# cure-lab/MagicDrive

Measured on AMD Instinct MI355X. Metric: 6-view scenes/sec at 224x400, 50-step DDIM, higher is better.
Workload: dtype bf16; 1 GPU; configs[1]: 6-view 224x400, text-only conditioning (camera_param=None -> CFG off), 50-step DDIM, bf16; scenes_per_gpu=64, ddim_steps=50, scheduler=ddim, parallelism=scene-sharded x1, hipgraph=True, streams=2, output_type=latent

## Files before the change

### include/mdx.h

```cpp
#ifndef MDX_H_
#define MDX_H_

#include <stdint.h>

#ifdef __cplusplus
extern "C" {
#endif

#define MDX_OK 0
#define MDX_EINVAL (-1)
#define MDX_ELAUNCH (-2)
#define MDX_EUNSUPPORTED (-3)

#define MDX_ABI_VERSION 12

#define MDX_EPI_NONE 0
#define MDX_EPI_GEGLU 1
#define MDX_EPI_SILU 2

typedef struct MdxGemmDesc {
    const void* A; const void* W; void* C; const void* R;
    const float* bias; const float* temb; const int32_t* sel_ptr; float* ws;
    int64_t M, N, K;
    int64_t lda, ldw, ldc, ldr;
// ... 46 lines not shown
    int64_t ldq, sQ, ldk, sK, ldv, sV, ldo, sO;
    double scale;
    int64_t joint;
    int64_t q_prescaled;
    int64_t causal;
    int64_t v_rowmajor;
} MdxAttnDesc;
int mdx_attention_bf16(const MdxAttnDesc* d, void* stream);

typedef struct MdxGroupNormDesc {
    const void* X; void* Y; const float* gamma; const float* beta;
    int64_t B, HW, C, G, ldx, ldy;
    double eps;
    int64_t silu;
    float* ws; int64_t ws_bytes;
} MdxGroupNormDesc;
int mdx_groupnorm_bf16(const MdxGroupNormDesc* d, void* stream);

typedef struct MdxLayerNormDesc {
    const void* X; void* Y; const float* gamma; const float* beta;
    int64_t M, C, ldx, ldy;
    double eps;
    int64_t reserved0;
} MdxLayerNormDesc;
int mdx_layernorm_bf16(const MdxLayerNormDesc* d, void* stream);

typedef struct MdxSoftmaxDesc {
    const float* X; void* Y;
    int64_t rows, T, ldx, ldy;
    double scale;
    int64_t reserved0;
} MdxSoftmaxDesc;
// ... 116 lines not shown
```

### magicdrive_amd/_lib.py

```python
from __future__ import annotations

import ctypes as C
import os
from typing import Dict, List, Tuple

_HERE = os.path.dirname(os.path.abspath(__file__))
LIB_PATH = os.environ.get("MDX_LIB_PATH") or os.path.join(_HERE, "libmdx.so")

ABI_VERSION = 12

OP_GEMM, OP_CONV, OP_CONV_DIRECT, OP_ATTN, OP_GROUPNORM, OP_LAYERNORM = 1, 2, 3, 4, 5, 6
OP_EW, OP_FOURIER, OP_GATHER, OP_TIMEEMB, OP_DDIM, OP_UNIPC, OP_SOFTMAX = 7, 8, 9, 10, 11, 12, 13
OP_BYTES = 512

EPI_NONE, EPI_GEGLU, EPI_SILU = 0, 1, 2
EW_ADD, EW_COPY, EW_UPSAMPLE, EW_NCHW_TO_NHWC, EW_NHWC_TO_NCHW, EW_SILU, EW_SCALE = 1, 2, 3, 4, 5, 6, 7

P, I, D = C.c_void_p, C.c_int64, C.c_double


def _struct(name: str, fields: List[Tuple[str, object]]):
    return type(name, (C.Structure,), {"_fields_": fields})


def _f(kind, names: str):
    return [(n, kind) for n in names.split()]


MdxGemmDesc = _struct("MdxGemmDesc", _f(P, "A W C R bias temb sel_ptr ws") + _f(I, "M N K lda ldw ldc ldr batch sA sW sC sR "
                      "temb_sel_stride temb_b_stride rows_per_b epilogue splitk c_is_f32 ws_bytes") + _f(P, "Vt") + _f(I, "vt_from vt_T vt_ld vt_stride")
                      + _f(D, "ln_eps") + _f(P, "ln_csum ln_scratch") + _f(P, "rowstat_out") + _f(I, "rowstat_parts") + _f(P, "ln_stats") + _f(I, "ln_stats_parts") + _f(P, "Wq"))
MdxConvDesc = _struct("MdxConvDesc", _f(P, "X Wt Y R bias temb sel_ptr ws") + _f(I, "B Hi Wi Cin Ho Wo Cout kh kw sh sw ph pw "
                      "ldx ldy ldr temb_sel_stride temb_b_stride epilogue splitk ws_bytes upsample2x"))
MdxConvDirectDesc = _struct("MdxConvDirectDesc", _f(P, "X Wt Y R bias temb sel_ptr reserved_p") + _f(I, "B Hi Wi Cin Ho Wo Cout kh kw sh sw ph pw "
                            "ldx ldy ldr temb_sel_stride temb_b_stride epilogue x_is_f32 y_is_f32 reserved0"))
MdxAttnDesc = _struct("MdxAttnDesc", _f(P, "Q K Vt O kvmap tk_dev") + _f(I, "B H Tq Tk d nsrc ldq sQ ldk sK ldv sV ldo sO")
                      + _f(D, "scale") + _f(I, "joint q_prescaled causal v_rowmajor"))
MdxGroupNormDesc = _struct("MdxGroupNormDesc", _f(P, "X Y gamma beta") + _f(I, "B HW C G ldx ldy") + _f(D, "eps") + _f(I, "silu") + _f(P, "ws") + _f(I, "ws_bytes"))
MdxLayerNormDesc = _struct("MdxLayerNormDesc", _f(P, "X Y gamma beta") + _f(I, "M C ldx ldy") + _f(D, "eps") + _f(I, "reserved0"))
MdxEwDesc = _struct("MdxEwDesc", _f(P, "X Y ymap xmap") + _f(I, "kind M C ldx ldy B Hi Wi Ho Wo x_is_f32 y_is_f32") + _f(D, "alpha"))
MdxFourierDesc = _struct("MdxFourierDesc", _f(P, "X Y mask null_feat") + _f(I, "n P F ldy"))
MdxGatherDesc = _struct("MdxGatherDesc", _f(P, "T Y idx mask null_row add") + _f(I, "n C ldt ldy n_rows add_period"))
MdxTimeEmbDesc = _struct("MdxTimeEmbDesc", _f(P, "t Y") + _f(I, "n dim flip_sin_to_cos ldy") + _f(D, "freq_shift max_period"))
MdxDdimDesc = _struct("MdxDdimDesc", _f(P, "x eps coef step_ptr x_in reserved_p") + _f(I, "n cfg") + _f(D, "guidance") + _f(I, "xin_c xin_ld")
                      + _f(P, "gv_cond gv_noise gv_mask") + _f(I, "gv_mode gv_view_elems gv_last_step"))
MdxUniPCDesc = _struct("MdxUniPCDesc", _f(P, "x eps coef step_ptr x_in x_last m1 m2") + _f(I, "n cfg") + _f(D, "guidance") + _f(I, "xin_c xin_ld")
                       + _f(P, "gv_cond gv_noise gv_mask") + _f(I, "gv_mode gv_view_elems gv_last_step"))

MdxSoftmaxDesc = _struct("MdxSoftmaxDesc", _f(P, "X Y") + _f(I, "rows T ldx ldy") + _f(D, "scale") + _f(I, "reserved0"))
DESC_OF_OP = {
    OP_GEMM: MdxGemmDesc, OP_CONV: MdxConvDesc, OP_CONV_DIRECT: MdxConvDirectDesc, OP_ATTN: MdxAttnDesc,
    OP_GROUPNORM: MdxGroupNormDesc, OP_LAYERNORM: MdxLayerNormDesc, OP_EW: MdxEwDesc, OP_FOURIER: MdxFourierDesc,
    OP_GATHER: MdxGatherDesc, OP_TIMEEMB: MdxTimeEmbDesc, OP_DDIM: MdxDdimDesc, OP_UNIPC: MdxUniPCDesc, OP_SOFTMAX: MdxSoftmaxDesc,
}
DTYPE_BF16, DTYPE_F16 = 0, 1
ENTRY_OF_OP = {
    OP_GEMM: "mdx_gemm_bf16", OP_CONV: "mdx_conv2d_bf16", OP_CONV_DIRECT: "mdx_conv2d_direct", OP_ATTN: "mdx_attention_bf16",
    OP_GROUPNORM: "mdx_groupnorm_bf16", OP_LAYERNORM: "mdx_layernorm_bf16", OP_EW: "mdx_elementwise",
    OP_FOURIER: "mdx_fourier_embed", OP_GATHER: "mdx_gather_rows", OP_TIMEEMB: "mdx_timestep_embedding", OP_DDIM: "mdx_cfg_ddim_step",
    OP_UNIPC: "mdx_cfg_unipc_step", OP_SOFTMAX: "mdx_softmax_rows",
}
def entry_name(opcode: int, dtype: int = DTYPE_BF16) -> str:
    n = ENTRY_OF_OP[opcode]
    if dtype == DTYPE_BF16:
        return n
    return (n[:-5] if n.endswith("_bf16") else n) + "_f16"


EXPORTS = sorted(set(ENTRY_OF_OP.values()) | {entry_name(o, DTYPE_F16) for o in ENTRY_OF_OP} | {
    "mdx_program_run", "mdx_graph_create", "mdx_graph_launch", "mdx_graph_destroy",
    "mdx_abi_version", "mdx_build_id", "mdx_last_error", "mdx_last_kernel", "mdx_device_info", "mdx_set_option", "mdx_get_option", "mdx_option_name"})


class MdxOp(C.Structure):
    _fields_ = [("opcode", I), ("dtype", I), ("desc", C.c_ubyte * (OP_BYTES - 16))]


assert C.sizeof(MdxOp) == OP_BYTES
for _d in DESC_OF_OP.values():
    assert C.sizeof(_d) <= OP_BYTES - 16 and C.sizeof(_d) % 8 == 0


class MdxError(RuntimeError):
    pass


# ... 24 lines not shown
    l.mdx_graph_launch.argtypes = [C.c_void_p, C.c_void_p]
    l.mdx_graph_destroy.restype = C.c_int
    l.mdx_graph_destroy.argtypes = [C.c_void_p]
    l.mdx_abi_version.restype = C.c_int
    l.mdx_last_error.restype = C.c_char_p
    l.mdx_build_id.restype = C.c_char_p
    l.mdx_last_kernel.restype = C.c_char_p
    l.mdx_device_info.restype = C.c_int
    l.mdx_device_info.argtypes = [C.POINTER(C.c_int64)]
    l.mdx_set_option.restype = C.c_int
    l.mdx_set_option.argtypes = [C.c_char_p, C.c_int64]
    l.mdx_get_option.restype = C.c_int
    l.mdx_get_option.argtypes = [C.c_char_p, C.POINTER(C.c_int64)]
    l.mdx_option_name.restype = C.c_char_p
    l.mdx_option_name.argtypes = [C.c_int64]
    if l.mdx_abi_version() != ABI_VERSION:
        raise MdxError(f"libmdx.so ABI {l.mdx_abi_version()} != expected {ABI_VERSION}")
    _LIB = l
    return l


def check(rc: int, what: str = "") -> None:
    if rc != 0:
        msg = lib().mdx_last_error()
        raise MdxError(f"{what} failed (rc={rc}): {msg.decode() if msg else ''}")


def call_op(opcode: int, desc: C.Structure, stream: int, dtype: int = DTYPE_BF16) -> None:
    name = entry_name(opcode, dtype)
    fn = getattr(lib(), name)
# ... 85 lines not shown
```

### magicdrive_amd/csrc/api.hip

```cpp
#include <cstring>
#include <mutex>
#include <set>
#include <utility>
#include "launch.h"
#include "options.h"
#include <atomic>
#include <cstdlib>

namespace mdx_rt {
char* error_buffer() {
    static thread_local char buf[512] = {0};
    return buf;
}
char* kernel_tag_buffer() {
    static thread_local char buf[128] = {0};
    return buf;
}
int ensure_dyn_smem(const void* kernel, size_t bytes, const char* what) {
    static std::mutex mu;
    static std::set<std::pair<const void*, int>> done;
    int dev = 0;
    hipError_t e = hipGetDevice(&dev);
    if (e != hipSuccess) return mdx::set_error(MDX_ELAUNCH, "hipGetDevice: %s", hipGetErrorString(e));
    std::lock_guard<std::mutex> lk(mu);
// ... 41 lines not shown

using namespace mdx;

extern "C" int mdx_set_option(const char* key, int64_t value) {
    const int i = find_opt(key);
    if (i < 0) return set_error(MDX_EINVAL, "mdx_set_option: unknown key '%s' (see magicdrive_amd/csrc/options.h)", key ? key : "(null)");
    g_opt[i].store(value, std::memory_order_relaxed);
    return MDX_OK;
}
extern "C" int mdx_get_option(const char* key, int64_t* value_out) {
    const int i = find_opt(key);
    if (i < 0 || !value_out) return set_error(MDX_EINVAL, "mdx_get_option: unknown key '%s'", key ? key : "(null)");
    *value_out = opt(i);
    return MDX_OK;
}
extern "C" const char* mdx_option_name(int64_t index) { return (index >= 0 && index < OPT_COUNT) ? kOptRows[index].key : nullptr; }

static int run_op(const MdxOp* op, hipStream_t st) {
    const void* d = op->desc;
    if (op->dtype == MDX_DTYPE_F16) {
        switch (op->opcode) {
            case MDX_OP_GEMM: return mdx_gemm_f16((const MdxGemmDesc*)d, st);
            case MDX_OP_CONV: return mdx_conv2d_f16((const MdxConvDesc*)d, st);
            case MDX_OP_CONV_DIRECT: return mdx_conv2d_direct_f16((const MdxConvDirectDesc*)d, st);
            case MDX_OP_ATTN: return mdx_attention_f16((const MdxAttnDesc*)d, st);
            case MDX_OP_GROUPNORM: return mdx_groupnorm_f16((const MdxGroupNormDesc*)d, st);
            case MDX_OP_LAYERNORM: return mdx_layernorm_f16((const MdxLayerNormDesc*)d, st);
            case MDX_OP_EW: return mdx_elementwise_f16((const MdxEwDesc*)d, st);
            case MDX_OP_FOURIER: return mdx_fourier_embed_f16((const MdxFourierDesc*)d, st);
            case MDX_OP_GATHER: return mdx_gather_rows_f16((const MdxGatherDesc*)d, st);
// ... 106 lines not shown
```

### magicdrive_amd/csrc/norm.hip

```cpp
#include "common.h"
#include "launch.h"
#include "options.h"

namespace mdx {

struct GNParams {
    const bf16_t* X; bf16_t* Y; const float* gamma; const float* beta;
    int B, HW, C, G; long ldx, ldy; float eps; int silu;
};

constexpr int GN_THREADS = 1024;
constexpr int GN_MAX_CPG = 2560;

__device__ __forceinline__ void block_sum2(float& a, float& b, float* red) {
    a = wave_sum(a);
    b = wave_sum(b);
    const int lane = threadIdx.x & 63, wave = threadIdx.x >> 6;
    __syncthreads();
    if (lane == 0) { red[wave] = a; red[16 + wave] = b; }
    __syncthreads();
    float ta = 0.f, tb = 0.f;
#pragma unroll
    for (int i = 0; i < GN_THREADS / 64; ++i) { ta += red[i]; tb += red[16 + i]; }
    a = ta; b = tb;
}

template <int VEC>
// ... 105 lines not shown
                *dptr = f2bf(o[0]);
            }
        }
        pxb += bigq; rb += bigr;
        if (rb >= vpp) { rb -= vpp; ++pxb; }
    }
}

struct GN2Params {
    const bf16_t* X; bf16_t* Y; const float* gamma; const float* beta; float* part;
    int B, HW, C, G, PCH, nchunk; long ldx, ldy; float eps; int silu;
    int rev;
    const float* stat;
};

constexpr int GN2_NT = 320;
constexpr int GN2_MAXC = 5120;
constexpr int GN2_U = 4;

__host__ __device__ __forceinline__ int gn2_rows(int C8) { return C8 >= 256 ? 1 : 256 / C8; }

template <int NCV>
__global__ __launch_bounds__(GN2_NT) void gn_stats_kernel(GN2Params p) {
    __shared__ float ls1[GN2_NT * 8 * NCV], ls2[GN2_NT * 8 * NCV];
    __shared__ float lpiv[256];
    const int chunk = p.rev ? p.nchunk - 1 - (int)blockIdx.x : (int)blockIdx.x, b = p.rev ? p.B - 1 - (int)blockIdx.y : (int)blockIdx.y, tid = threadIdx.x;
    const int px0 = chunk * p.PCH;
    const int npx = min(p.PCH, p.HW - px0);
    const int C8 = p.C / 8, cpg = p.C / p.G;
    const int rows = gn2_rows(C8);
    const bf16_t* xb = p.X + ((long)b * p.HW + px0) * p.ldx;
    if (tid < p.G) lpiv[tid] = bf2f(xb[tid * cpg]);
    __syncthreads();
    const int r0 = NCV == 1 ? tid / C8 : 0;
    const bool active = NCV == 1 ? r0 < rows : true;
// ... 126 lines not shown
#pragma unroll
            for (int k = 0; k < NCV; ++k) {
                float o[8];
#pragma unroll
                for (int e = 0; e < 8; ++e) {
                    float y = __builtin_fmaf(bf2f(f[u][k].h[e]), sc[k][e], sh[k][e]);
                    if (p.silu) y = silu_f(y);
                    o[e] = y;
                }
                uint4 w; w.x = pack2bf(o[0], o[1]); w.y = pack2bf(o[2], o[3]); w.z = pack2bf(o[4], o[5]); w.w = pack2bf(o[6], o[7]);
                if (px + u * rows < npx && cc[k] < C8) *(uint4*)(yb + (long)(px + u * rows) * ldy + cc[k] * 8) = w;
            }
    }
}

struct LNParams {
    const bf16_t* X; bf16_t* Y; const float* gamma; const float* beta;
    int M, C; long ldx, ldy; float eps;
};

template <int MAXV, int RPW, bool AFFINE>
__global__ __launch_bounds__(256) void layernorm_kernel(LNParams p) {
    const int lane = threadIdx.x & 63;
    const int row0 = (blockIdx.x * 4 + (threadIdx.x >> 6)) * RPW;
    if (row0 >= p.M) return;
    const int nv = p.C / 8;
    float v[RPW][MAXV][8];
    float s1[RPW];
    Frag8 f[RPW][MAXV];
#pragma unroll
// ... 79 lines not shown
extern "C" int mdx_groupnorm_bf16(const MdxGroupNormDesc* d, void* stream) {
    if (!d || !d->X || !d->Y || !d->gamma || !d->beta) return set_error(MDX_EINVAL, "mdx_groupnorm_bf16: null operand");
    if (d->G <= 0 || d->C % d->G) return set_error(MDX_EINVAL, "groupnorm: C=%ld not divisible by G=%ld", (long)d->C, (long)d->G);
    const char* op = "mdx_groupnorm_bf16";
    MDX_NEED(need_int(op, "B", d->B)); MDX_NEED(need_int(op, "HW", d->HW)); MDX_NEED(need_int(op, "C", d->C)); MDX_NEED(need_int(op, "G", d->G));
    MDX_NEED(need_aligned(op, "gamma", d->gamma, 16)); MDX_NEED(need_aligned(op, "beta", d->beta, 16)); MDX_NEED(need_aligned(op, "ws", d->ws, 16));
    MDX_NEED(need_aligned(op, "X", d->X, 2)); MDX_NEED(need_aligned(op, "Y", d->Y, 2));
    if (d->C <= 0 || d->ldx < d->C || d->ldy < d->C) return set_error(MDX_EINVAL, "%s: need 0 < C <= ldx, ldy", op);
    if (d->B <= 0 || d->HW <= 0) return MDX_OK;
    GNParams p;
    p.X = (const bf16_t*)d->X; p.Y = (bf16_t*)d->Y; p.gamma = d->gamma; p.beta = d->beta;
    p.B = (int)d->B; p.HW = (int)d->HW; p.C = (int)d->C; p.G = (int)d->G; p.ldx = d->ldx; p.ldy = d->ldy;
    p.eps = (float)d->eps; p.silu = (int)d->silu;
    const int cpg = p.C / p.G;
    hipStream_t st = (hipStream_t)stream;
    const int two_stage = (int)opt(OPT_GN_TWO_STAGE);
    const long elems = (long)p.HW * p.C;
    const int nt_ws = (p.C % 8 == 0) ? ((p.C / 8) > GN2_NT ? GN2_NT : gn2_rows(p.C / 8) * (p.C / 8)) : 0;
    const bool small = (long)p.B * elems <= opt(OPT_GN_ONE_KERNEL_ELEMS);
    if (two_stage && !small && d->ws && elems >= 32768 && p.C % 8 == 0 && p.C <= GN2_MAXC && p.G <= nt_ws && p.ldx % 8 == 0 && p.ldy % 8 == 0 &&
        ((uintptr_t)p.X & 15) == 0 && ((uintptr_t)p.Y & 15) == 0) {
        GN2Params q;
        q.X = p.X; q.Y = p.Y; q.gamma = p.gamma; q.beta = p.beta; q.part = (float*)d->ws;
        q.B = p.B; q.HW = p.HW; q.C = p.C; q.G = p.G; q.ldx = p.ldx; q.ldy = p.ldy; q.eps = p.eps; q.silu = p.silu;
        q.rev = (int)opt(OPT_GN_REVERSE);
        q.stat = nullptr;
        const int C8 = p.C / 8, rows = gn2_rows(C8);
        const int nt = C8 > GN2_NT ? GN2_NT : rows * C8;
        int target = (int)(4096 / p.B); if (target < 1) target = 1;
        int pch = (p.HW + target - 1) / target;
        if (pch < rows * GN2_U) pch = rows * GN2_U;
        pch = (pch + rows - 1) / rows * rows;
        if (pch > p.HW) pch = p.HW;
        q.PCH = pch;
        q.nchunk = (p.HW + q.PCH - 1) / q.PCH;
        const long part_bytes = (long)p.B * q.nchunk * p.G * 3 * (long)sizeof(float);
        if (part_bytes <= d->ws_bytes) {
            dim3 grid2(q.nchunk, p.B);
            if (C8 > GN2_NT) hipLaunchKernelGGL(gn_stats_kernel<2>, grid2, dim3(nt), 0, st, q);
            else hipLaunchKernelGGL(gn_stats_kernel<1>, grid2, dim3(nt), 0, st, q);
            int rc = check_launch("gn_stats_kernel", false);
            if (rc) return rc;
            q.stat = nullptr;
            const long stat_bytes = (long)p.B * p.G * 2 * (long)sizeof(float);
            const long fin = opt(OPT_GN_FINALIZE_CHUNKS);
            if (fin > 0 && q.nchunk > fin && part_bytes + stat_bytes <= d->ws_bytes) {
                float* stat = (float*)((char*)d->ws + part_bytes);
                hipLaunchKernelGGL(gn_finalize_kernel, dim3(p.G, p.B), dim3(64), 0, st, q.part, stat, q.nchunk, p.G, p.eps);
                rc = check_launch("gn_finalize_kernel", false);
                if (rc) return rc;
                q.stat = stat;
            }
            if (C8 > GN2_NT) hipLaunchKernelGGL(gn_apply_kernel<2>, grid2, dim3(nt), 0, st, q);
            else hipLaunchKernelGGL(gn_apply_kernel<1>, grid2, dim3(nt), 0, st, q);
            return check_launch("gn_stats_kernel+gn_apply_kernel");
        }
    }
    if (cpg > GN_MAX_CPG) return set_error(MDX_EUNSUPPORTED, "groupnorm: %d channels per group (at most %d outside the two-stage path)", cpg, GN_MAX_CPG);
    int vec = 1;
    for (int v = 8; v > 1; v >>= 1) {
        if (cpg % v == 0 && p.ldx % v == 0 && p.ldy % v == 0 && ((uintptr_t)p.X % (2 * v)) == 0 && ((uintptr_t)p.Y % (2 * v)) == 0) { vec = v; break; }
    }
    dim3 grid(p.G, p.B);
    switch (vec) {
        case 8: hipLaunchKernelGGL(groupnorm_kernel<8>, grid, dim3(GN_THREADS), 0, st, p); break;
        case 4: hipLaunchKernelGGL(groupnorm_kernel<4>, grid, dim3(GN_THREADS), 0, st, p); break;
        case 2: hipLaunchKernelGGL(groupnorm_kernel<2>, grid, dim3(GN_THREADS), 0, st, p); break;
        default: hipLaunchKernelGGL(groupnorm_kernel<1>, grid, dim3(GN_THREADS), 0, st, p); break;
    }
    return check_launch("groupnorm_kernel");
}

namespace mdx {
// ... 94 lines not shown
```

### magicdrive_amd/csrc/options.h

```cpp
#pragma once
#include <cstdint>

namespace mdx_rt {
int64_t opt(int id);
}

namespace mdx {

#define MDX_OPTIONS(X) \
    X(ATTN_SWZ, 2, "XCD-aware block order of attention.hip: 0 off, 1 per (view, head), 2 per view (all heads of a view on one XCD)") \
    X(ATTN_NW4_BLOCKS, 256L, "attention.hip: 4-wave workgroups from this many blocks") \
    X(ATTN_NW8_BLOCKS, (1L << 40), "attention.hip: 8-wave workgroups from this many blocks") \
    X(ATTN_NW, 0, "force the waves per workgroup of attention.hip (0 = heuristic)") \
    X(ATTN2, 1, "attention2.hip for head dim 40") \
    X(ATTN3, 0, "only in `make ATTN3=1` builds: tools/attn3/attention3.hip (permute-free P, QK of the next kv tile beside this tile's softmax) for the head-dim-40 FOLD launches: self, cross-view, joint") \
    X(ATTN3_WGS, 0, "attention3.hip: persistent workgroups per XCD (0 = automatic: two per CU)") \
    X(ATTN2_PF, 1, "attention2.hip, head dim 40 FOLD 32-query form: permute-free P (PV on 32x32x16 MFMAs, K rows permuted so that a lane's scores are its PV operand)") \
    X(ATTN2_D80, 2, "attention2.hip for head dim 80: 0 never, 1 always, 2 only the two-source cross-view form") \
    X(ATTN2_FOLD, 1, "attention2.hip: subtract the running maximum inside the QK MFMA when Q is pre-scaled (head dim 40)") \
    X(ATTN2_RES, 1, "attention2.hip: kv sequences of <= 3 tiles (text context) resident in LDS, one workgroup per (view, head) walks the query blocks: 0 off, 1 for launches of >= 1024 (view, head) pairs, 2 whenever supported") \
    X(ATTN2_VIEWMAP, 1, "attention2.hip block order: 1 = all heads and query blocks of a view on one XCD (a row's 128-byte lines are shared by the heads), 0 = per (view, head)") \
    X(ATTN2_QT, 0, "32-query tiles per wave in attention2.hip: 0 = automatic (2; 1 for one-source FOLD launches), 1 / 2 = force") \
    X(CONV_OUT_WS, 1, "direct conv with Cout <= 4 and a long K (conv_out): weight-stationary K-parallel kernel (weights in registers, 16 pixels per wave)") \
    X(GEMM_SWZ, 1, "XCD-aware tile order of the generic kernel") \
// ... 7 lines not shown
    X(XL_K320, 0, "let XL take the K = 320 projections from gemm_ws.hip") \
    X(XL_MIN_TILES, 64, "fewest 256-row tiles an XL launch must have (round 6: 64; 160 until then — 2...8 scenes per call are 2-6 % faster with the lower bound, 12+ scenes and 1 scene do not care: profiles/r06_lat1_small_grids.log)") \
    X(XL_BN, 0, "force an XL tile width (160 / 256 / 320; 0 = cost model)") \
    X(XL_GEGLU320, 0, "K = 320 GEGLU on the 256-wide XL tile instead of gemm_ws.hip") \
    X(GEMM_BM256, 0, "generic 256x128 8-wave tile from M >= value (0 = never)") \
    X(GEMM_TIMING, 0, "s_memtime stamps of the generic kernel into the op workspace") \
    X(GEMM_BK, 64, "generic tile slab depth (64 or 32)") \
    X(GEMM_FLATTEN, 1, "batched shared-A GEMM as ONE col_split XL launch") \
    X(CONV_CIMAJOR, 1, "channel-block-major K order of implicit-GEMM convs") \
    X(WS_SLOTS, 512, "workgroup slots the gemm_ws M walkers are sized for") \
    X(XL_TIMING, 0, "per-workgroup s_memtime stamps into the op workspace") \
    X(GN_REVERSE, 1, "two-stage GroupNorm: statistics pass reads the tensor back to front (Infinity-Cache reuse between producer / passes)") \
    X(GN_FINALIZE_CHUNKS, 16, "two-stage GroupNorm: with more chunks per image than this the chunk partials are combined once by gn_finalize_kernel (0 = always in the apply pass)") \
    X(GN_ONE_KERNEL_ELEMS, (4L << 20), "GroupNorm tensors of at most this many elements (all images) take the one-launch kernel (one workgroup per (image, group)) instead of the two streaming passes") \
    X(GN_TWO_STAGE, 1, "streaming two-stage GroupNorm for maps >= 32768 elements") \
    X(XL_PERSIST, 1, "256x256 XL GEMMs (plain / GEGLU, optional residual) on the persistent kernel gemm_xlp_kernel") \
    X(XD, 0, "W-direct persistent GEMM (gemm_xd.hip: weights global -> registers, finished tile stored under the next tile's main loop) for the 256x256 XL GEMMs whose descriptor carries Wq (K % 128 == 0, K >= 640); bit-identical to gemm_xlp_kernel, measured 0.89-1.04x of it (profiles/r06_xd_ab.log): off by default") \
    X(XL_RASTER, 2, "XL tile order: 0 row-major, 1 XCD-strided M-tiles, 2 XCD-blocked (M-group x N-group panels per XCD)") \
    X(XL_GM, 0, "XL_RASTER 2: force the M-tiles per panel (0 = cost model, xl_layout.h: raster_shape)") \
    X(XL_GN, 0, "XL_RASTER 2: force the N-tiles per panel (0 = cost model)") \
    X(STREAMS, 2, "host side (pipeline): HIP streams a pipe() call spreads its scene chunks over (chunks of >= 16 scenes, one plan + hipGraph each)") \
    X(PLAN_CACHE, 6, "host side (pipeline): sampler plans (captured graphs + buffers) kept per pipeline (LRU); a multi-stream call pins one plan per chunk") \
    X(CHECK_TIMESTEPS, 0, "host side (schedulers): 1 = a device-resident timestep that is not in the scheduler's list raises (one sync per step) instead of poisoning the sample with NaN") \
    X(LN_FUSE, 1, "MdxGemmDesc.ln_eps: 1 = gemm_ws.hip normalises the rows in-kernel, 0 = always normalise into ln_scratch first (A/B)") \
    X(LN_STATS, 1, "MdxGemmDesc.rowstat_out / ln_stats: 1 = row statistics travel from the producer's store phase to the fused LayerNorm, 0 = round-5 behaviour (nothing emitted, in-kernel sums, GEGLU through ln_scratch) (A/B)")

enum Opt : int {
#define MDX_OPT_ENUM(key, dflt, doc) OPT_##key,
    MDX_OPTIONS(MDX_OPT_ENUM)
#undef MDX_OPT_ENUM
// ... 7 lines not shown
```

### magicdrive_amd/engine.py

```python
from __future__ import annotations

from typing import Dict, List, Optional, Sequence, Tuple

import torch

from . import _lib as L
from . import ops as O
from . import packing as PK
from .networks.spec import heads_at

BF16, F32 = torch.bfloat16, torch.float32


def q_prescale(head_dim: int) -> float:
    return float(head_dim) ** -0.5 * 1.4426950408889634


class PackedNet:

    def __init__(self, sd: Dict[str, torch.Tensor], device, dtype=BF16):
        assert dtype in (torch.bfloat16, torch.float16), "the kernels take bf16 or fp16 operands (fp32 accumulate)"
        self.sd = sd
        self.device = device
        self.dtype = dtype
# ... 234 lines not shown

    def emit(self, op):
        self.ops.append(op)
        return op

    def new(self, B, H, W, C) -> Act:
        return Act(self.pool.get((B * H * W, C)), B, H, W, C)

    def free(self, a):
        if isinstance(a, ActSlice):
            return
        self.pool.put(a.t if isinstance(a, Act) else a)

    def groupnorm(self, net, pre, x: Act, eps, silu, name) -> Act:
        y = self.new(x.B, x.H, x.W, x.C)
        self.emit(O.GroupNorm(x.btc, y.btc, net.vec(pre + "weight"), net.vec(pre + "bias"), self.groups, eps, silu, ws=self.ws, name=name))
        return y

    def layernorm(self, net, pre, x: torch.Tensor, name) -> torch.Tensor:
        y = self.pool.get(tuple(x.shape))
        self.emit(O.LayerNorm(x, y, net.vec(pre + "weight"), net.vec(pre + "bias"), 1e-5, name=name))
        return y

    @staticmethod
    def wq_of(W: torch.Tensor, M: int, epilogue: int) -> Optional[torch.Tensor]:
        if W.dim() != 2 or not W.is_contiguous() or epilogue not in (L.EPI_NONE, L.EPI_GEGLU) or not L.get_option("XD"):
            return None
        N, K = W.shape
        if K % 128 or K < 640 or N % 16 or ((M + 255) // 256) * ((N + 255) // 256) < 512:
            return None
        wq = getattr(W, "_mdx_wq", None)
# ... 325 lines not shown
```

### magicdrive_amd/flops.py

```python
from __future__ import annotations

from collections import defaultdict
from typing import Dict, Iterable

from . import ops as O


def kernel_family(op) -> str:
    if isinstance(op, O.Conv):
        return "conv_direct" if op.direct else "gemm_conv_kernel<conv>"
    if isinstance(op, O.Gemm):
        return "gemm_conv_kernel<gemm>"
    if isinstance(op, O.Attn):
        return "attn_kernel"
    if isinstance(op, O.GroupNorm):
        return "groupnorm_kernel"
    if isinstance(op, O.LayerNorm):
        return "layernorm_kernel"
    return "elementwise"


def op_flops(op) -> float:
    if isinstance(op, O.Gemm):
        C = op.C
        batch = C.shape[0] if C.dim() == 3 else 1
        M = C.shape[-2]
        N = op.W.shape[-2]
        K = op.W.shape[-1]
        return 2.0 * batch * M * N * K
    if isinstance(op, O.Conv):
        B, Ho, Wo, Cout = op.Y.shape
# ... 33 lines not shown
```

### magicdrive_amd/ops.py

```python
from __future__ import annotations

from dataclasses import dataclass, field
from typing import Optional

import torch

from . import _lib as L

BF16 = torch.bfloat16
F16 = torch.float16
H16 = (BF16, F16)
F32 = torch.float32


def _p(t: Optional[torch.Tensor]):
    return None if t is None else t.data_ptr()


def _chk(cond: bool, msg: str):
    if not cond:
        raise ValueError(msg)


def _rows2d(t: torch.Tensor):
# ... 260 lines not shown
        _chk(self.nsrc >= 1 and (self.nsrc <= 8 if self.joint else self.nsrc <= 2), f"attn {self.name}: nsrc={self.nsrc} (joint={self.joint})")
        return self.opcode, d


@dataclass
class GroupNorm:
    X: torch.Tensor
    Y: torch.Tensor
    gamma: torch.Tensor
    beta: torch.Tensor
    groups: int
    eps: float
    silu: bool = False
    ws: Optional[torch.Tensor] = None
    name: str = ""
    opcode = L.OP_GROUPNORM

    def lower(self):
        B, HW, Cc = self.X.shape
        _chk(self.X.stride(2) == 1 and self.Y.stride(2) == 1 and self.Y.shape == self.X.shape, f"gn {self.name}: layout")
        _chk(B == 1 or (self.X.stride(0) == HW * self.X.stride(1) and self.Y.stride(0) == HW * self.Y.stride(1)), f"gn {self.name}: batch stride")
        _chk(self.gamma.dtype == F32 and self.beta.dtype == F32 and self.gamma.numel() == Cc, f"gn {self.name}: affine")
        d = L.MdxGroupNormDesc()
        d.X, d.Y, d.gamma, d.beta = _p(self.X), _p(self.Y), _p(self.gamma), _p(self.beta)
        d.B, d.HW, d.C, d.G, d.ldx, d.ldy = B, HW, Cc, self.groups, self.X.stride(1), self.Y.stride(1)
        d.eps, d.silu = float(self.eps), int(self.silu)
        if self.ws is not None:
            d.ws = _p(self.ws); d.ws_bytes = self.ws.numel() * self.ws.element_size()
        return self.opcode, d


@dataclass
class LayerNorm:
    X: torch.Tensor
    Y: torch.Tensor
    gamma: torch.Tensor
    beta: torch.Tensor
    eps: float = 1e-5
    name: str = ""
    opcode = L.OP_LAYERNORM

    def lower(self):
        M, Cc, ldx = _rows2d(self.X)
        M2, C2, ldy = _rows2d(self.Y)
# ... 290 lines not shown
```

Baseline: 7.527 scenes/s.

## Add register-resident one-pass GroupNorm kernel for large-batch UNet norms

Adds a GroupNorm kernel where one 1024-thread workgroup keeps a slice of groups for one image in registers. It computes statistics with a shifted-mean reduction, then applies normalization and optional SiLU from those registers. This replaces the two-stage stats and apply path, which reads the input twice and writes partials to a workspace. Routing logic moves to a shared header, and a query entry point lets Python tooling see which path runs. The risk is high register pressure and low occupancy from 1024-thread blocks holding up to 16 uint4 fragments each.

```diff
diff --git a/include/mdx.h b/include/mdx.h
--- a/include/mdx.h
+++ b/include/mdx.h
@@ -84,8 +84,10 @@
     double eps;
     int64_t silu;
     float* ws; int64_t ws_bytes;
+    int64_t resident;
 } MdxGroupNormDesc;
 int mdx_groupnorm_bf16(const MdxGroupNormDesc* d, void* stream);
+int mdx_groupnorm_route(const MdxGroupNormDesc* d);
 
 typedef struct MdxLayerNormDesc {
     const void* X; void* Y; const float* gamma; const float* beta;
diff --git a/magicdrive_amd/_lib.py b/magicdrive_amd/_lib.py
--- a/magicdrive_amd/_lib.py
+++ b/magicdrive_amd/_lib.py
@@ -36,7 +36,7 @@
                             "ldx ldy ldr temb_sel_stride temb_b_stride epilogue x_is_f32 y_is_f32 reserved0"))
 MdxAttnDesc = _struct("MdxAttnDesc", _f(P, "Q K Vt O kvmap tk_dev") + _f(I, "B H Tq Tk d nsrc ldq sQ ldk sK ldv sV ldo sO")
                       + _f(D, "scale") + _f(I, "joint q_prescaled causal v_rowmajor"))
-MdxGroupNormDesc = _struct("MdxGroupNormDesc", _f(P, "X Y gamma beta") + _f(I, "B HW C G ldx ldy") + _f(D, "eps") + _f(I, "silu") + _f(P, "ws") + _f(I, "ws_bytes"))
+MdxGroupNormDesc = _struct("MdxGroupNormDesc", _f(P, "X Y gamma beta") + _f(I, "B HW C G ldx ldy") + _f(D, "eps") + _f(I, "silu") + _f(P, "ws") + _f(I, "ws_bytes resident"))
 MdxLayerNormDesc = _struct("MdxLayerNormDesc", _f(P, "X Y gamma beta") + _f(I, "M C ldx ldy") + _f(D, "eps") + _f(I, "reserved0"))
 MdxEwDesc = _struct("MdxEwDesc", _f(P, "X Y ymap xmap") + _f(I, "kind M C ldx ldy B Hi Wi Ho Wo x_is_f32 y_is_f32") + _f(D, "alpha"))
 MdxFourierDesc = _struct("MdxFourierDesc", _f(P, "X Y mask null_feat") + _f(I, "n P F ldy"))
@@ -53,6 +53,7 @@
     OP_GROUPNORM: MdxGroupNormDesc, OP_LAYERNORM: MdxLayerNormDesc, OP_EW: MdxEwDesc, OP_FOURIER: MdxFourierDesc,
     OP_GATHER: MdxGatherDesc, OP_TIMEEMB: MdxTimeEmbDesc, OP_DDIM: MdxDdimDesc, OP_UNIPC: MdxUniPCDesc, OP_SOFTMAX: MdxSoftmaxDesc,
 }
+GN_ONE_LAUNCH, GN_TWO_STAGE, GN_RESIDENT = 0, 1, 2
 DTYPE_BF16, DTYPE_F16 = 0, 1
 ENTRY_OF_OP = {
     OP_GEMM: "mdx_gemm_bf16", OP_CONV: "mdx_conv2d_bf16", OP_CONV_DIRECT: "mdx_conv2d_direct", OP_ATTN: "mdx_attention_bf16",
@@ -69,7 +70,7 @@
 
 EXPORTS = sorted(set(ENTRY_OF_OP.values()) | {entry_name(o, DTYPE_F16) for o in ENTRY_OF_OP} | {
     "mdx_program_run", "mdx_graph_create", "mdx_graph_launch", "mdx_graph_destroy",
-    "mdx_abi_version", "mdx_build_id", "mdx_last_error", "mdx_last_kernel", "mdx_device_info", "mdx_set_option", "mdx_get_option", "mdx_option_name"})
+    "mdx_abi_version", "mdx_build_id", "mdx_last_error", "mdx_last_kernel", "mdx_device_info", "mdx_set_option", "mdx_get_option", "mdx_option_name", "mdx_groupnorm_route"})
 
 
 class MdxOp(C.Structure):
@@ -124,6 +125,8 @@
     l.mdx_get_option.argtypes = [C.c_char_p, C.POINTER(C.c_int64)]
     l.mdx_option_name.restype = C.c_char_p
     l.mdx_option_name.argtypes = [C.c_int64]
+    l.mdx_groupnorm_route.restype = C.c_int
+    l.mdx_groupnorm_route.argtypes = [C.c_void_p]
     if l.mdx_abi_version() != ABI_VERSION:
         raise MdxError(f"libmdx.so ABI {l.mdx_abi_version()} != expected {ABI_VERSION}")
     _LIB = l
diff --git a/magicdrive_amd/csrc/api.hip b/magicdrive_amd/csrc/api.hip
--- a/magicdrive_amd/csrc/api.hip
+++ b/magicdrive_amd/csrc/api.hip
@@ -4,6 +4,7 @@
 #include <utility>
 #include "launch.h"
 #include "options.h"
+#include "gn_route.h"
 #include <atomic>
 #include <cstdlib>
 
@@ -79,6 +80,24 @@
     *value_out = opt(i);
     return MDX_OK;
 }
+extern "C" int mdx_groupnorm_route(const MdxGroupNormDesc* d) {
+    if (!d || !d->X || !d->Y || !d->gamma || !d->beta) return mdx::set_error(MDX_EINVAL, "mdx_groupnorm_route: null operand");
+    if (d->G <= 0 || d->C <= 0 || d->C % d->G || d->B <= 0 || d->HW <= 0) return mdx::set_error(MDX_EINVAL, "mdx_groupnorm_route: need B, HW, C, G > 0 and C %% G == 0");
+    for (int64_t v : {d->B, d->HW, d->C, d->G}) if (v > 0x7fffffffL) return mdx::set_error(MDX_EINVAL, "mdx_groupnorm_route: B, HW, C, G must fit a 32-bit int");
+    if (d->ldx < d->C || d->ldy < d->C) return mdx::set_error(MDX_EINVAL, "mdx_groupnorm_route: need C <= ldx, ldy");
+    if (((uintptr_t)d->gamma | (uintptr_t)d->beta | (uintptr_t)d->ws) & 15) return mdx::set_error(MDX_EINVAL, "mdx_groupnorm_route: gamma, beta, ws must be 16-byte aligned");
+    if (((uintptr_t)d->X | (uintptr_t)d->Y) & 1) return mdx::set_error(MDX_EINVAL, "mdx_groupnorm_route: X, Y must be 2-byte aligned");
+    mdx_route::GnRouteIn ri;
+    ri.B = d->B; ri.HW = d->HW; ri.C = d->C; ri.G = d->G; ri.ldx = d->ldx; ri.ldy = d->ldy;
+    ri.has_ws = d->ws != nullptr; ri.ws_bytes = d->ws_bytes;
+    ri.x_al16 = ((uintptr_t)d->X & 15) == 0; ri.y_al16 = ((uintptr_t)d->Y & 15) == 0;
+    ri.resident = d->resident != 0;
+    const mdx_route::GnRouteOpts ro = {mdx_rt::opt(mdx::OPT_GN_TWO_STAGE), mdx_rt::opt(mdx::OPT_GN_ONE_KERNEL_ELEMS), mdx_rt::opt(mdx::OPT_GN_RESIDENT)};
+    const mdx_route::GnRoute rt = mdx_route::gn_route(ri, ro);
+    if (rt.err) return mdx::set_error(MDX_EUNSUPPORTED, "groupnorm: more than %d channels per group outside the two-stage path", mdx_route::GN_MAX_CPG);
+    return rt.main;
+}
+
 extern "C" const char* mdx_option_name(int64_t index) { return (index >= 0 && index < OPT_COUNT) ? kOptRows[index].key : nullptr; }
 
 static int run_op(const MdxOp* op, hipStream_t st) {
diff --git a/magicdrive_amd/csrc/gn_route.h b/magicdrive_amd/csrc/gn_route.h
--- /dev/null
+++ b/magicdrive_amd/csrc/gn_route.h
@@ -0,0 +1,94 @@
+#pragma once
+
+#if defined(__HIPCC__) || defined(__HIP__)
+#define MDX_GN_HD __host__ __device__ __forceinline__
+#else
+#define MDX_GN_HD inline
+#endif
+
+namespace mdx_route {
+
+constexpr int GNR_THREADS = 1024;
+constexpr int GNR_MAX_U = 16;
+constexpr int GNR_MAX_SC = 2560;
+constexpr int GNR_MAX_GROUPS = 32;
+constexpr int GNR_MIN_SV = 10;
+
+constexpr int GNR_MIN_IMAGES = 192;
+
+constexpr int GN2_NT = 320;
+constexpr int GN2_MAXC = 5120;
+constexpr int GN2_U = 4;
+constexpr int GN_MAX_CPG = 2560;
+
+MDX_GN_HD int gn2_rows(int C8) { return C8 >= 256 ? 1 : 256 / C8; }
+
+struct GnRouteIn {
+    long B, HW, C, G, ldx, ldy;
+    bool has_ws; long ws_bytes;
+    bool x_al16, y_al16;
+    bool resident;
+};
+struct GnRouteOpts { long GN_TWO_STAGE, GN_ONE_KERNEL_ELEMS, GN_RESIDENT; };
+
+enum GnMain { GN_ONE_LAUNCH = 0, GN_TWO_STAGE = 1, GN_RESIDENT = 2 };
+
+struct GnRoute {
+    int main;
+    int err;
+    int pch, nchunk;
+    int ns, sc, sv, rows, U;
+};
+
+inline bool gn_resident_fit(const GnRouteIn& p, GnRoute& r) {
+    if (p.G <= 0 || p.C % p.G || p.C % 8 || p.ldx % 8 || p.ldy % 8 || !p.x_al16 || !p.y_al16) return false;
+    const long cpg = p.C / p.G;
+    if (cpg < 8 || p.HW * p.ldx >= (1L << 30) || p.HW * p.ldy >= (1L << 30)) return false;
+    for (long ns = 1; ns <= p.G; ++ns) {
+        if (p.G % ns) continue;
+        const long gs = p.G / ns, sc = gs * cpg;
+        if (sc % 8) continue;
+        const long sv = sc / 8;
+        if (sv < GNR_MIN_SV) break;
+        if (sc > GNR_MAX_SC || gs > GNR_MAX_GROUPS || sv > GNR_THREADS) continue;
+        const long rows = GNR_THREADS / sv;
+        const long U = (p.HW + rows - 1) / rows;
+        if (U > GNR_MAX_U) continue;
+        if (p.B * ns > 0x7ffffff0L) return false;
+        r.ns = (int)ns; r.sc = (int)sc; r.sv = (int)sv; r.rows = (int)rows; r.U = (int)U;
+        return true;
+    }
+    return false;
+}
+
+inline GnRoute gn_route(const GnRouteIn& p, const GnRouteOpts& o) {
+    GnRoute r = {};
+    r.main = GN_ONE_LAUNCH;
+    const long elems = p.HW * p.C, cpg = p.G > 0 ? p.C / p.G : 0;
+    const long C8 = p.C / 8;
+    const long nt_ws = (p.C % 8 == 0) ? (C8 > GN2_NT ? GN2_NT : gn2_rows((int)C8) * C8) : 0;
+    const bool small = p.B * elems <= o.GN_ONE_KERNEL_ELEMS;
+    if (o.GN_TWO_STAGE && !small && p.has_ws && elems >= 32768 && p.C % 8 == 0 && p.C <= GN2_MAXC && p.G <= nt_ws && p.ldx % 8 == 0 && p.ldy % 8 == 0 &&
+        p.x_al16 && p.y_al16) {
+        const long rows = gn2_rows((int)C8);
+        long target = 4096 / p.B; if (target < 1) target = 1;
+        long pch = (p.HW + target - 1) / target;
+        if (pch < rows * GN2_U) pch = rows * GN2_U;
+        pch = (pch + rows - 1) / rows * rows;
+        if (pch > p.HW) pch = p.HW;
+        const long nchunk = (p.HW + pch - 1) / pch;
+        if (p.B * nchunk * p.G * 3 * 4 <= p.ws_bytes) {
+            r.main = GN_TWO_STAGE; r.pch = (int)pch; r.nchunk = (int)nchunk;
+            if (p.resident && (o.GN_RESIDENT >= 2 || (o.GN_RESIDENT == 1 && p.B >= GNR_MIN_IMAGES)) && gn_resident_fit(p, r)) r.main = GN_RESIDENT;
+            return r;
+        }
+    }
+    if (cpg > GN_MAX_CPG) r.err = 1;
+    return r;
+}
+
+inline const char* gn_route_tag(int main) {
+    return main == GN_RESIDENT ? "gn_resident_kernel" : main == GN_TWO_STAGE ? "gn_stats_kernel+gn_apply_kernel" : "groupnorm_kernel";
+}
+
+}
diff --git a/magicdrive_amd/csrc/norm.hip b/magicdrive_amd/csrc/norm.hip
--- a/magicdrive_amd/csrc/norm.hip
+++ b/magicdrive_amd/csrc/norm.hip
@@ -1,6 +1,8 @@
 #include "common.h"
 #include "launch.h"
 #include "options.h"
+#include "gn_route.h"
+#include <type_traits>
 
 namespace mdx {
 
@@ -10,7 +12,7 @@
 };
 
 constexpr int GN_THREADS = 1024;
-constexpr int GN_MAX_CPG = 2560;
+using mdx_route::GN_MAX_CPG;
 
 __device__ __forceinline__ void block_sum2(float& a, float& b, float* red) {
     a = wave_sum(a);
@@ -146,11 +148,10 @@
     const float* stat;
 };
 
-constexpr int GN2_NT = 320;
-constexpr int GN2_MAXC = 5120;
-constexpr int GN2_U = 4;
-
-__host__ __device__ __forceinline__ int gn2_rows(int C8) { return C8 >= 256 ? 1 : 256 / C8; }
+using mdx_route::GN2_NT;
+using mdx_route::GN2_U;
+using mdx_route::gn2_rows;
+
 
 template <int NCV>
 __global__ __launch_bounds__(GN2_NT) void gn_stats_kernel(GN2Params p) {
@@ -307,6 +308,109 @@
     }
 }
 
+struct GNRParams {
+    const bf16_t* X; bf16_t* Y; const float* gamma; const float* beta;
+    int B, HW, C, G, ns, sc, sv, rows; long ldx, ldy; float eps; int silu;
+};
+
+constexpr int GNR_THREADS = mdx_route::GNR_THREADS;
+
+template <int U>
+__global__ __launch_bounds__(GNR_THREADS) void gn_resident_kernel(GNRParams p) {
+    __shared__ float part[4][GNR_THREADS];
+    __shared__ float gb[2][mdx_route::GNR_MAX_SC];
+    __shared__ float gstat[2][mdx_route::GNR_MAX_GROUPS];
+    const int total = p.B * p.ns, per = (total + 7) >> 3;
+    const int unit = ((int)blockIdx.x & 7) * per + ((int)blockIdx.x >> 3);
+    if (unit >= total) return;
+    const int b = unit / p.ns, s = unit - b * p.ns;
+    const int tid = threadIdx.x, lane = tid & 63, wave = tid >> 6;
+    const int cpg = p.C / p.G, gs = p.sc / cpg, sv = p.sv, rows = p.rows;
+    const bf16_t* xb = p.X + (long)b * p.HW * p.ldx + (long)s * p.sc;
+    bf16_t* yb = p.Y + (long)b * p.HW * p.ldy + (long)s * p.sc;
+    for (int c = tid; c < p.sc; c += GNR_THREADS) { gb[0][c] = p.gamma[s * p.sc + c]; gb[1][c] = p.beta[s * p.sc + c]; }
+    float pvw[2];
+#pragma unroll
+    for (int k = 0; k < 2; ++k) pvw[k] = bf2f(xb[min(wave + 16 * k, gs - 1) * cpg]);
+    const int r0 = tid / sv, cv = tid - r0 * sv;
+    const bool active = r0 < rows;
+    const int gA = active ? (cv * 8) / cpg : 0;
+    const int nA = min(8, (gA + 1) * cpg - cv * 8);
+    const int gB = min(gA + 1, gs - 1);
+    Frag8 f[U];
+    const int xo = r0 * (int)p.ldx + cv * 8, xstep = rows * (int)p.ldx, xlast = (p.HW - 1) * (int)p.ldx + cv * 8;
+    const int nv = active ? (p.HW - r0 + rows - 1) / rows : 0;
+    if (active) {
+        const float pvA = bf2f(xb[gA * cpg]), pvB = bf2f(xb[gB * cpg]);
+#pragma unroll
+        for (int u = 0; u < U; ++u) f[u].u = *(const uint4*)((const char*)xb + (unsigned)(u < nv ? xo + u * xstep : xlast) * 2u);
+        float s1[8], s2[8];
+#pragma unroll
+        for (int e = 0; e < 8; ++e) { s1[e] = 0.f; s2[e] = 0.f; }
+#pragma unroll
+        for (int u = 0; u < U; ++u)
+            if (u < nv) {
+#pragma unroll
+                for (int e = 0; e < 8; ++e) { const float d = bf2f(f[u].h[e]) - (e < nA ? pvA : pvB); s1[e] += d; s2[e] = __builtin_fmaf(d, d, s2[e]); }
+            }
+        float a1 = 0.f, a2 = 0.f, b1 = 0.f, b2 = 0.f;
+#pragma unroll
+        for (int e = 0; e < 8; ++e) {
+            if (e < nA) { a1 += s1[e]; a2 += s2[e]; } else { b1 += s1[e]; b2 += s2[e]; }
+        }
+        part[0][tid] = a1; part[1][tid] = a2; part[2][tid] = b1; part[3][tid] = b2;
+    }
+    __syncthreads();
+#pragma unroll
+    for (int k = 0; k < 2; ++k) {
+        const int g = wave + 16 * k;
+        if (g < gs) {
+            const int cv_lo = (g * cpg) / 8, cv_hi = ((g + 1) * cpg - 1) / 8, ncv = cv_hi - cv_lo + 1, nit = rows * ncv;
+            float t1 = 0.f, t2 = 0.f;
+            for (int i = lane; i < nit; i += 64) {
+                const int r = i / ncv, cvv = cv_lo + (i - r * ncv), t = r * sv + cvv;
+                const int q = (cvv * 8) / cpg == g ? 0 : 2;
+                t1 += part[q][t]; t2 += part[q + 1][t];
+            }
+            t1 = wave_sum(t1); t2 = wave_sum(t2);
+            if (lane == 0) {
+                const float n = (float)p.HW * (float)cpg;
+                const float md = t1 / n;
+                gstat[0][g] = pvw[k] + md;
+                gstat[1][g] = rsqrtf(fmaxf(t2 / n - md * md, 0.f) + p.eps);
+            }
+        }
+    }
+    __syncthreads();
+    if (!active) return;
+#pragma unroll
+    for (int u = 0; u < U; ++u) asm volatile("" : "+v"(f[u].u.x), "+v"(f[u].u.y), "+v"(f[u].u.z), "+v"(f[u].u.w));
+    int yo = r0 * (int)p.ldy + cv * 8, ystep = rows * (int)p.ldy;
+    asm volatile("" : "+v"(yo), "+s"(ystep));
+    float sc[8], sh[8];
+#pragma unroll
+    for (int e = 0; e < 8; ++e) {
+        const int g = e < nA ? gA : gB;
+        const float w = gstat[1][g] * gb[0][cv * 8 + e];
+        sc[e] = w; sh[e] = gb[1][cv * 8 + e] - gstat[0][g] * w;
+    }
+    auto apply = [&](auto silu) {
+#pragma unroll
+        for (int u = 0; u < U; ++u) {
+            float o[8];
+#pragma unroll
+            for (int e = 0; e < 8; ++e) {
+                float y = __builtin_fmaf(bf2f(f[u].h[e]), sc[e], sh[e]);
+                if constexpr (decltype(silu)::value) y = y * __builtin_amdgcn_rcpf(1.0f + __builtin_amdgcn_exp2f(y * -1.4426950408889634f));
+                o[e] = y;
+            }
+            uint4 w; w.x = pack2bf(o[0], o[1]); w.y = pack2bf(o[2], o[3]); w.z = pack2bf(o[4], o[5]); w.w = pack2bf(o[6], o[7]);
+            if (u < nv) *(uint4*)((char*)yb + (unsigned)(yo + u * ystep) * 2u) = w;
+        }
+    };
+    if (p.silu) apply(std::true_type{}); else apply(std::false_type{});
+}
+
 struct LNParams {
     const bf16_t* X; bf16_t* Y; const float* gamma; const float* beta;
     int M, C; long ldx, ldy; float eps;
@@ -416,12 +520,27 @@
     p.eps = (float)d->eps; p.silu = (int)d->silu;
     const int cpg = p.C / p.G;
     hipStream_t st = (hipStream_t)stream;
-    const int two_stage = (int)opt(OPT_GN_TWO_STAGE);
-    const long elems = (long)p.HW * p.C;
-    const int nt_ws = (p.C % 8 == 0) ? ((p.C / 8) > GN2_NT ? GN2_NT : gn2_rows(p.C / 8) * (p.C / 8)) : 0;
-    const bool small = (long)p.B * elems <= opt(OPT_GN_ONE_KERNEL_ELEMS);
-    if (two_stage && !small && d->ws && elems >= 32768 && p.C % 8 == 0 && p.C <= GN2_MAXC && p.G <= nt_ws && p.ldx % 8 == 0 && p.ldy % 8 == 0 &&
-        ((uintptr_t)p.X & 15) == 0 && ((uintptr_t)p.Y & 15) == 0) {
+    mdx_route::GnRouteIn ri;
+    ri.B = d->B; ri.HW = d->HW; ri.C = d->C; ri.G = d->G; ri.ldx = d->ldx; ri.ldy = d->ldy;
+    ri.has_ws = d->ws != nullptr; ri.ws_bytes = d->ws_bytes;
+    ri.x_al16 = ((uintptr_t)p.X & 15) == 0; ri.y_al16 = ((uintptr_t)p.Y & 15) == 0;
+    ri.resident = d->resident != 0;
+    const mdx_route::GnRouteOpts ro = {opt(OPT_GN_TWO_STAGE), opt(OPT_GN_ONE_KERNEL_ELEMS), opt(OPT_GN_RESIDENT)};
+    const mdx_route::GnRoute rt = mdx_route::gn_route(ri, ro);
+    if (rt.main == mdx_route::GN_RESIDENT) {
+        GNRParams q;
+        q.X = p.X; q.Y = p.Y; q.gamma = p.gamma; q.beta = p.beta;
+        q.B = p.B; q.HW = p.HW; q.C = p.C; q.G = p.G; q.ns = rt.ns; q.sc = rt.sc; q.sv = rt.sv; q.rows = rt.rows;
+        q.ldx = p.ldx; q.ldy = p.ldy; q.eps = p.eps; q.silu = p.silu;
+        const dim3 grid((unsigned)(((long)p.B * rt.ns + 7) / 8 * 8));
+        if (rt.U <= 4) hipLaunchKernelGGL(gn_resident_kernel<4>, grid, dim3(GNR_THREADS), 0, st, q);
+        else if (rt.U <= 8) hipLaunchKernelGGL(gn_resident_kernel<8>, grid, dim3(GNR_THREADS), 0, st, q);
+        else if (rt.U <= 12) hipLaunchKernelGGL(gn_resident_kernel<12>, grid, dim3(GNR_THREADS), 0, st, q);
+        else if (rt.U <= 14) hipLaunchKernelGGL(gn_resident_kernel<14>, grid, dim3(GNR_THREADS), 0, st, q);
+        else hipLaunchKernelGGL(gn_resident_kernel<16>, grid, dim3(GNR_THREADS), 0, st, q);
+        return check_launch(mdx_route::gn_route_tag(rt.main));
+    }
+    if (rt.main == mdx_route::GN_TWO_STAGE) {
         GN2Params q;
         q.X = p.X; q.Y = p.Y; q.gamma = p.gamma; q.beta = p.beta; q.part = (float*)d->ws;
         q.B = p.B; q.HW = p.HW; q.C = p.C; q.G = p.G; q.ldx = p.ldx; q.ldy = p.ldy; q.eps = p.eps; q.silu = p.silu;
@@ -429,36 +548,28 @@
         q.stat = nullptr;
         const int C8 = p.C / 8, rows = gn2_rows(C8);
         const int nt = C8 > GN2_NT ? GN2_NT : rows * C8;
-        int target = (int)(4096 / p.B); if (target < 1) target = 1;
-        int pch = (p.HW + target - 1) / target;
-        if (pch < rows * GN2_U) pch = rows * GN2_U;
-        pch = (pch + rows - 1) / rows * rows;
-        if (pch > p.HW) pch = p.HW;
-        q.PCH = pch;
-        q.nchunk = (p.HW + q.PCH - 1) / q.PCH;
+        q.PCH = rt.pch;
+        q.nchunk = rt.nchunk;
         const long part_bytes = (long)p.B * q.nchunk * p.G * 3 * (long)sizeof(float);
-        if (part_bytes <= d->ws_bytes) {
-            dim3 grid2(q.nchunk, p.B);
-            if (C8 > GN2_NT) hipLaunchKernelGGL(gn_stats_kernel<2>, grid2, dim3(nt), 0, st, q);
-            else hipLaunchKernelGGL(gn_stats_kernel<1>, grid2, dim3(nt), 0, st, q);
-            int rc = check_launch("gn_stats_kernel", false);
+        dim3 grid2(q.nchunk, p.B);
+        if (C8 > GN2_NT) hipLaunchKernelGGL(gn_stats_kernel<2>, grid2, dim3(nt), 0, st, q);
+        else hipLaunchKernelGGL(gn_stats_kernel<1>, grid2, dim3(nt), 0, st, q);
+        int rc = check_launch("gn_stats_kernel", false);
+        if (rc) return rc;
+        const long stat_bytes = (long)p.B * p.G * 2 * (long)sizeof(float);
+        const long fin = opt(OPT_GN_FINALIZE_CHUNKS);
+        if (fin > 0 && q.nchunk > fin && part_bytes + stat_bytes <= d->ws_bytes) {
+            float* stat = (float*)((char*)d->ws + part_bytes);
+            hipLaunchKernelGGL(gn_finalize_kernel, dim3(p.G, p.B), dim3(64), 0, st, q.part, stat, q.nchunk, p.G, p.eps);
+            rc = check_launch("gn_finalize_kernel", false);
             if (rc) return rc;
-            q.stat = nullptr;
-            const long stat_bytes = (long)p.B * p.G * 2 * (long)sizeof(float);
-            const long fin = opt(OPT_GN_FINALIZE_CHUNKS);
-            if (fin > 0 && q.nchunk > fin && part_bytes + stat_bytes <= d->ws_bytes) {
-                float* stat = (float*)((char*)d->ws + part_bytes);
-                hipLaunchKernelGGL(gn_finalize_kernel, dim3(p.G, p.B), dim3(64), 0, st, q.part, stat, q.nchunk, p.G, p.eps);
-                rc = check_launch("gn_finalize_kernel", false);
-                if (rc) return rc;
-                q.stat = stat;
-            }
-            if (C8 > GN2_NT) hipLaunchKernelGGL(gn_apply_kernel<2>, grid2, dim3(nt), 0, st, q);
-            else hipLaunchKernelGGL(gn_apply_kernel<1>, grid2, dim3(nt), 0, st, q);
-            return check_launch("gn_stats_kernel+gn_apply_kernel");
-        }
-    }
-    if (cpg > GN_MAX_CPG) return set_error(MDX_EUNSUPPORTED, "groupnorm: %d channels per group (at most %d outside the two-stage path)", cpg, GN_MAX_CPG);
+            q.stat = stat;
+        }
+        if (C8 > GN2_NT) hipLaunchKernelGGL(gn_apply_kernel<2>, grid2, dim3(nt), 0, st, q);
+        else hipLaunchKernelGGL(gn_apply_kernel<1>, grid2, dim3(nt), 0, st, q);
+        return check_launch(mdx_route::gn_route_tag(rt.main));
+    }
+    if (rt.err) return set_error(MDX_EUNSUPPORTED, "groupnorm: %d channels per group (at most %d outside the two-stage path)", cpg, GN_MAX_CPG);
     int vec = 1;
     for (int v = 8; v > 1; v >>= 1) {
         if (cpg % v == 0 && p.ldx % v == 0 && p.ldy % v == 0 && ((uintptr_t)p.X % (2 * v)) == 0 && ((uintptr_t)p.Y % (2 * v)) == 0) { vec = v; break; }
diff --git a/magicdrive_amd/csrc/options.h b/magicdrive_amd/csrc/options.h
--- a/magicdrive_amd/csrc/options.h
+++ b/magicdrive_amd/csrc/options.h
@@ -45,6 +45,7 @@
     X(GN_FINALIZE_CHUNKS, 16, "two-stage GroupNorm: with more chunks per image than this the chunk partials are combined once by gn_finalize_kernel (0 = always in the apply pass)") \
     X(GN_ONE_KERNEL_ELEMS, (4L << 20), "GroupNorm tensors of at most this many elements (all images) take the one-launch kernel (one workgroup per (image, group)) instead of the two streaming passes") \
     X(GN_TWO_STAGE, 1, "streaming two-stage GroupNorm for maps >= 32768 elements") \
+    X(GN_RESIDENT, 1, "resident one-pass GroupNorm (gn_resident_kernel) for ops that ask for it (MdxGroupNormDesc.resident) and fit: 0 never (such ops take the two-stage path again: A/B), 1 in calls of >= 192 images (the measured batches), 2 whenever a slice fits") \
     X(XL_PERSIST, 1, "256x256 XL GEMMs (plain / GEGLU, optional residual) on the persistent kernel gemm_xlp_kernel") \
     X(XD, 0, "W-direct persistent GEMM (gemm_xd.hip: weights global -> registers, finished tile stored under the next tile's main loop) for the 256x256 XL GEMMs whose descriptor carries Wq (K % 128 == 0, K >= 640); bit-identical to gemm_xlp_kernel, measured 0.89-1.04x of it (profiles/r06_xd_ab.log): off by default") \
     X(XL_RASTER, 2, "XL tile order: 0 row-major, 1 XCD-strided M-tiles, 2 XCD-blocked (M-group x N-group panels per XCD)") \
diff --git a/magicdrive_amd/engine.py b/magicdrive_amd/engine.py
--- a/magicdrive_amd/engine.py
+++ b/magicdrive_amd/engine.py
@@ -272,7 +272,8 @@
 
     def groupnorm(self, net, pre, x: Act, eps, silu, name) -> Act:
         y = self.new(x.B, x.H, x.W, x.C)
-        self.emit(O.GroupNorm(x.btc, y.btc, net.vec(pre + "weight"), net.vec(pre + "bias"), self.groups, eps, silu, ws=self.ws, name=name))
+        self.emit(O.GroupNorm(x.btc, y.btc, net.vec(pre + "weight"), net.vec(pre + "bias"), self.groups, eps, silu, ws=self.ws, name=name,
+                              resident=True))
         return y
 
     def layernorm(self, net, pre, x: torch.Tensor, name) -> torch.Tensor:
diff --git a/magicdrive_amd/flops.py b/magicdrive_amd/flops.py
--- a/magicdrive_amd/flops.py
+++ b/magicdrive_amd/flops.py
@@ -3,6 +3,7 @@
 from collections import defaultdict
 from typing import Dict, Iterable
 
+from . import _lib as L
 from . import ops as O
 
 
@@ -14,7 +15,7 @@
     if isinstance(op, O.Attn):
         return "attn_kernel"
     if isinstance(op, O.GroupNorm):
-        return "groupnorm_kernel"
+        return "gn_resident_kernel" if op.resident and op.route() == L.GN_RESIDENT else "groupnorm_kernel"
     if isinstance(op, O.LayerNorm):
         return "layernorm_kernel"
     return "elementwise"
diff --git a/magicdrive_amd/ops.py b/magicdrive_amd/ops.py
--- a/magicdrive_amd/ops.py
+++ b/magicdrive_amd/ops.py
@@ -1,5 +1,6 @@
 from __future__ import annotations
 
+import ctypes as C
 from dataclasses import dataclass, field
 from typing import Optional
 
@@ -298,6 +299,7 @@
     silu: bool = False
     ws: Optional[torch.Tensor] = None
     name: str = ""
+    resident: bool = False
     opcode = L.OP_GROUPNORM
 
     def lower(self):
@@ -311,7 +313,13 @@
         d.eps, d.silu = float(self.eps), int(self.silu)
         if self.ws is not None:
             d.ws = _p(self.ws); d.ws_bytes = self.ws.numel() * self.ws.element_size()
-        return self.opcode, d
+        d.resident = int(self.resident)
+        return self.opcode, d
+
+    def route(self) -> int:
+        rc = L.lib().mdx_groupnorm_route(C.byref(self.lower()[1]))
+        L.check(0 if rc >= 0 else rc, f"mdx_groupnorm_route {self.name}")
+        return rc
 
 
 @dataclass
```

Measured after the change: 7.635 scenes/s (median of 6 runs). 1.4% higher.
